# edwindn/rl-agent-for-qubit-array-tuning

Hardware: AMD Instinct MI355X
Metric: env steps/sec (batched 8-dot 64x64 CSD solves) (higher is better)
Workload: dtype f64; 1 GPU; 8-dot array, 4096 parallel envs per GPU, 64x64 CSD, deterministic physics (latching/noise off), 50-step episodes, staggered phases: 820 episode resets (new device + first observation) inside the timed region, synthetic CNN outputs; n_dots=8, envs_per_gpu=4096, resolution=64

## Files before the change

### __graft_entry__.py

```python
import os
import subprocess
import sys

ROOT = os.path.dirname(os.path.abspath(__file__))
PKG = os.path.join(ROOT, "rl-agent-for-qubit-array-tuning_amd")
for _p in (PKG, os.path.join(ROOT, "oracle"), os.path.join(ROOT, "tests")):
    if _p not in sys.path:
        sys.path.insert(0, _p)


def build() -> None:
    csrc = os.path.join(PKG, "csrc")
    subprocess.check_call(["make", "-C", csrc, "libqdsim.so"])
    subprocess.check_call(["make", "-C", os.path.join(ROOT, "tests", "hosttest"), "libqdsim_hosttest.so", "qd_scratch_asan"])
    subprocess.check_call(["make", "-C", os.path.join(ROOT, "tests", "hosttest_wave"), "libqdsim_hosttest_wave.so"])
    subprocess.check_call(["make", "-C", os.path.join(ROOT, "tests", "hosttest_gs"), "libqdsim_hosttest_gs.so"])
    subprocess.check_call(["make", "-C", os.path.join(ROOT, "tests", "hosttest_prune"), "libqdsim_hosttest_prune.so"])
    subprocess.check_call(["make", "-C", os.path.join(ROOT, "tests", "hosttest_points"), "libqdsim_hosttest_points.so"])
    subprocess.check_call(["make", "-C", os.path.join(ROOT, "tests", "hosttest_latch"), "libqdsim_hosttest_latch.so"])
    subprocess.check_call(["make", "-C", os.path.join(ROOT, "tests", "hosttest_scan"), "libqdsim_hosttest_scan.so"])
    subprocess.check_call(["make", "-C", os.path.join(ROOT, "tests", "hosttest_affine"), "libqdsim_hosttest_affine.so"])
    subprocess.check_call(["make", "-C", os.path.join(ROOT, "tests", "hosttest_line"), "libqdsim_hosttest_line.so"])
    subprocess.check_call(["make", "-C", os.path.join(ROOT, "tests", "hosttest_grid"), "libqdsim_hosttest_grid.so", "qd_grid_asan"])
    subprocess.check_call(["make", "-C", os.path.join(ROOT, "tests", "hosttest_tile"), "libqdsim_hosttest_tile.so", "qd_tile_asan"])
    subprocess.check_call(["make", "-C", os.path.join(ROOT, "tests", "hosttest_insert"), "all", "qd_insert_asan"])
    subprocess.check_call(["make", "-C", os.path.join(ROOT, "tests", "hosttest_closed"), "libqdsim_hosttest_closed.so", "qd_closed_asan"])
    subprocess.check_call(["make", "-C", os.path.join(ROOT, "tests", "hosttest_levels"), "libqdsim_hosttest_levels.so", "qd_levels_asan"])
    subprocess.check_call(["make", "-C", os.path.join(ROOT, "tests", "hosttest_thermal"), "libqdsim_hosttest_thermal.so", "qd_thermal_asan"])
    subprocess.check_call(["make", "-C", os.path.join(ROOT, "tests", "hosttest_thermal_blocks"), "libqdsim_hosttest_thermal_blocks.so",
                           "qd_thermal_blocks_asan"])
    subprocess.check_call(["make", "-C", os.path.join(ROOT, "tests", "hosttest_levels_blocks"), "libqdsim_hosttest_levels_blocks.so",
                           "qd_levels_blocks_asan"])
    subprocess.check_call(["make", "-C", os.path.join(ROOT, "tests", "hosttest_response"), "libqdsim_hosttest_response.so",
                           "qd_response_asan"])
    subprocess.check_call(["make", "-C", os.path.join(ROOT, "tests", "hosttest_response_blocks"), "libqdsim_hosttest_response_blocks.so",
                           "qd_response_blocks_asan"])
    subprocess.check_call(["make", "-C", os.path.join(ROOT, "tests", "gputest_eig"), "libqdsim_gputest_eig.so"])
    subprocess.check_call(["make", "-C", os.path.join(ROOT, "tests", "gputest_thermal_blocks"), "libqdsim_gputest_thermal_blocks.so"])
    subprocess.check_call(["make", "-C", os.path.join(ROOT, "tests", "gputest_levels_blocks"), "libqdsim_gputest_levels_blocks.so"])
    subprocess.check_call(["make", "-C", os.path.join(ROOT, "tests", "gputest_response"), "libqdsim_gputest_response.so"])
    subprocess.check_call(["make", "-C", os.path.join(ROOT, "tests", "gputest_response_blocks"), "libqdsim_gputest_response_blocks.so"])
    subprocess.check_call(["make", "-C", os.path.join(ROOT, "oracle"), "libqdoracle.so"])
    import qadapt_hip
    from qadapt_hip import _lib
    L = _lib.lib()
    missing = [n for n in _lib.EXPORTS + _lib.EXPORTS_WITH_DIGITS if not hasattr(L, n)]
    if missing:
        raise RuntimeError(f"libqdsim.so lacks symbols: {missing}")


def smoke() -> None:
    import numpy as np
    import torch
    import qd_oracle as O
    import helpers as H
    from qadapt_hip.vec_env import VecQuantumDeviceEnv, SyntheticCapacitanceModel

    assert torch.cuda.is_available(), "smoke() needs the MI355X"
    N, R, B, seed = 4, 16, 2, 2024
    env = VecQuantumDeviceEnv(B, num_dots=N, resolution=R, seed=seed, validate=True,
                              capacitance_model=SyntheticCapacitanceModel(3))
    rng = np.random.default_rng(0)
    C = N - 1
    v0 = rng.normal(0, 0.1, (B, C, 3)).astype(np.float32); l0 = rng.uniform(-6, -2, (B, C, 3)).astype(np.float32)
    obs = env.reset(cnn_outputs=(torch.as_tensor(v0).cuda(), torch.as_tensor(l0).cuda()))
    act = rng.uniform(-1, 1, (B, 2 * N - 1)).astype(np.float32)
    v1 = rng.normal(0, 0.1, (B, C, 3)).astype(np.float32); l1 = rng.uniform(-6, -2, (B, C, 3)).astype(np.float32)
    obs, rew, term, trunc = env.step(torch.as_tensor(act).cuda(),
                                     cnn_outputs=(torch.as_tensor(v1).cuda(), torch.as_tensor(l1).cuda()))
    img = obs["image"].cpu().numpy()
    raw, _ = env.raw()
    for e in range(B):
        oe = O.OracleEnv(N, R)
        oe.reset(O.sample_episode(np.random.default_rng(seed + e), N), v0[e], l0[e])
        oobs, (gr, br), _, _ = oe.step(act[e, :N], act[e, N:], v1[e], l1[e])
        r = rew[e].cpu().numpy()
        assert np.allclose(r[:N], gr, rtol=1e-9) and np.allclose(r[N:], br, rtol=1e-9), "reward mismatch"
        H.image_parity(oe, img[e], raw[e])
    env.close()
    print("smoke ok: 4-dot 16x16 batched step matches the oracle")


if __name__ == "__main__":
    build()
    if len(sys.argv) > 1 and sys.argv[1] == "smoke":
        smoke()
```

### rl-agent-for-qubit-array-tuning_amd/csrc/qd_tile.h

```cpp
#pragma once
#include "qd_pixel.h"
#include "qd_groundstate.h"

#define QD_FL_BIAS 0x7FFF
QD_HD bool qd_fl_packable(int fl) { return (unsigned)fl <= (unsigned)QD_FL_BIAS; }
QD_HD uint32_t qd_fl_pack(int fl) { return (uint32_t)fl | ((uint32_t)(QD_FL_BIAS - fl) << 16); }
QD_HD uint32_t qd_fl_pkmin(uint32_t a, uint32_t b) {
#if defined(__HIP_DEVICE_COMPILE__)
    typedef unsigned short u16x2 __attribute__((ext_vector_type(2)));
    return __builtin_bit_cast(uint32_t, __builtin_elementwise_min(__builtin_bit_cast(u16x2, a), __builtin_bit_cast(u16x2, b)));
#else
    const uint32_t la = a & 0xFFFFu, lb = b & 0xFFFFu, ha = a >> 16, hb = b >> 16;
    return (la < lb ? la : lb) | ((ha < hb ? ha : hb) << 16);
#endif
}
QD_HD void qd_fl_unpack(uint32_t w, int& mn, int& mx) { mn = (int)(w & 0xFFFFu); mx = QD_FL_BIAS - (int)(w >> 16); }

#ifndef QD_TILE_RESCAN8
#define QD_TILE_RESCAN8 1
#endif
template <int KC, bool FILL, bool RESCAN8 = (QD_TILE_RESCAN8 != 0)>
QD_HD void qd_tile_select(int nS, int nSfront, int scap, const uint32_t* scode, const double* sD, const double* sa, const double* sb,
                          double xs, double ys, uint32_t blo, uint32_t bhi, double* ke, uint16_t* kid,
                          double& maxE_out, int& maxS_out, int& maxG_out, int& count_out, double& eout_out) {
    constexpr int NG = KC / 8;
    double gE[4] = {-INFINITY, -INFINITY, -INFINITY, -INFINITY}; int gS[4] = {0, 8, 16, 24};
    double maxE = -INFINITY; int maxS = 0, maxG = 0, count = 0;
    double eout = INFINITY;
    int si0 = 0, nfree = 0;
    if (FILL && nSfront >= KC) {
#pragma unroll
        for (int g = 0; g < NG; ++g) {
            double me = -INFINITY; int ms = g * 8;
#pragma unroll
            for (int t = 0; t < 8; ++t) {
                const int s = g * 8 + t;
                const double en = fma(xs, sa[s], fma(ys, sb[s], sD[s]));
                ke[s * 64] = en; kid[s * 64] = (uint16_t)s;
                if (en > me) { me = en; ms = s; }
            }
            gE[g] = me; gS[g] = ms;
        }
        maxE = gE[0]; maxS = gS[0]; maxG = 0;
#pragma unroll
        for (int g = 1; g < NG; ++g) if (gE[g] > maxE) { maxE = gE[g]; maxS = gS[g]; maxG = g; }
        count = KC; si0 = KC; nfree = nSfront;
    }
    for (int si = si0; si < nS; ++si) {
        const int s = si < nSfront ? si : scap - 1 - (si - nSfront);
        const uint32_t code = scode[s];
        const bool valid = (si < nfree) ||
                           (((((code | 0x88888888u) - blo) & 0x88888888u) == 0x88888888u) &&
                            ((((bhi | 0x88888888u) - code) & 0x88888888u) == 0x88888888u));
        const double en = fma(xs, sa[s], fma(ys, sb[s], sD[s]));
        if (!valid) continue;
        if (count < KC) {
            ke[count * 64] = en; kid[count * 64] = (uint16_t)s;
            count++;
            if (count == KC) {
#pragma unroll
                for (int g = 0; g < NG; ++g) {
                    double me = -INFINITY; int ms = g * 8;
#pragma unroll
                    for (int t = 0; t < 8; ++t) { const double v = ke[(g * 8 + t) * 64]; if (v > me) { me = v; ms = g * 8 + t; } }
                    gE[g] = me; gS[g] = ms;
                }
                maxE = gE[0]; maxS = gS[0]; maxG = 0;
#pragma unroll
                for (int g = 1; g < NG; ++g) if (gE[g] > maxE) { maxE = gE[g]; maxS = gS[g]; maxG = g; }
            }
        } else if (en < maxE) {
            eout = fmin(eout, maxE);
            ke[maxS * 64] = en; kid[maxS * 64] = (uint16_t)s;
            {
                double me = -INFINITY; int ms = maxG * 8;
                if constexpr (RESCAN8) {
                    double v[8];
#pragma unroll
                    for (int t = 0; t < 8; ++t) v[t] = ke[(maxG * 8 + t) * 64];
#if defined(__HIP_DEVICE_COMPILE__)
                    __builtin_amdgcn_sched_barrier(0);
#endif
#pragma unroll
                    for (int t = 0; t < 8; ++t) if (v[t] > me) { me = v[t]; ms = maxG * 8 + t; }
                } else {
#pragma unroll
                    for (int t = 0; t < 8; ++t) { const double v = ke[(maxG * 8 + t) * 64]; if (v > me) { me = v; ms = maxG * 8 + t; } }
                }
#pragma unroll
                for (int g = 0; g < NG; ++g) if (g == maxG) { gE[g] = me; gS[g] = ms; }
            }
            maxE = gE[0]; maxS = gS[0]; maxG = 0;
#pragma unroll
            for (int g = 1; g < NG; ++g) if (gE[g] > maxE) { maxE = gE[g]; maxS = gS[g]; maxG = g; }
        } else {
            eout = fmin(eout, en);
        }
    }
    maxE_out = maxE; maxS_out = maxS; maxG_out = maxG; count_out = count; eout_out = eout;
}

#if defined(__HIPCC__)

#ifndef QD_TILE_PG_INTERLEAVED
#define QD_TILE_PG_INTERLEAVED 1
#endif
#ifndef QD_TILE_DPP
#define QD_TILE_DPP 1
#endif
#ifndef QD_TILE_FILL
#define QD_TILE_FILL 1
#endif

#ifndef QD_T_FCAP
#define QD_T_FCAP 832
#endif
#ifndef QD_T_SCAP
#define QD_T_SCAP 383
#endif
#define QD_T_REDO (-1)

struct QdTileLds {
    double m[QD_MAXN], g[QD_MAXN], lamx[QD_MAXN], lamy[QD_MAXN], tail[QD_MAXN], sla[QD_MAXN], slb[QD_MAXN], q[QD_MAXN];
    int lo[QD_MAXN], nd[QD_MAXN], cg[QD_MAXN];
    int optval[QD_MAXN][4];
    union {
        struct { double pn[2][QD_T_FCAP]; uint32_t code[2][QD_T_FCAP]; } f;
        struct { double e[QD_K][64]; uint16_t id[QD_K][64]; } k;
    } u;
    double sD[QD_T_SCAP], sa[QD_T_SCAP], sb[QD_T_SCAP];
    uint32_t scode[QD_T_SCAP];
#if defined(QD_TILE_PAD_LDS)
    char pad[QD_TILE_PAD_LDS];
#endif
};

__device__ __forceinline__ double qd_rl(double v, int lane) {
    const unsigned long long u = (unsigned long long)__double_as_longlong(v);
    const unsigned lo = (unsigned)__builtin_amdgcn_readlane((int)(unsigned)u, lane);
    const unsigned hi = (unsigned)__builtin_amdgcn_readlane((int)(unsigned)(u >> 32), lane);
    return __longlong_as_double((long long)(((unsigned long long)hi << 32) | lo));
}
template <int CTRL>
__device__ __forceinline__ int qd_dpp_i32(int v) { return __builtin_amdgcn_update_dpp(v, v, CTRL, 0xF, 0xF, false); }
#define QD_ROW_ALLREDUCE(v, OP, DPP)                                                                                   \
    v = OP(v, DPP<0xB1>(v));                                                               \
    v = OP(v, DPP<0x4E>(v));                                                               \
    v = OP(v, DPP<0x141>(v));                                                                     \
    v = OP(v, DPP<0x140>(v))
__device__ __forceinline__ int qd_wmin_i(int v) {
#if QD_TILE_DPP
    QD_ROW_ALLREDUCE(v, min, qd_dpp_i32);
    return min(min(__builtin_amdgcn_readlane(v, 0), __builtin_amdgcn_readlane(v, 16)),
               min(__builtin_amdgcn_readlane(v, 32), __builtin_amdgcn_readlane(v, 48)));
#else
#pragma unroll
    for (int o = 32; o > 0; o >>= 1) v = min(v, __shfl_xor(v, o, 64));
    return __builtin_amdgcn_readfirstlane(v);
#endif
}
__device__ __forceinline__ int qd_wmax_i(int v) {
#if QD_TILE_DPP
    QD_ROW_ALLREDUCE(v, max, qd_dpp_i32);
    return max(max(__builtin_amdgcn_readlane(v, 0), __builtin_amdgcn_readlane(v, 16)),
               max(__builtin_amdgcn_readlane(v, 32), __builtin_amdgcn_readlane(v, 48)));
#else
#pragma unroll
    for (int o = 32; o > 0; o >>= 1) v = max(v, __shfl_xor(v, o, 64));
    return __builtin_amdgcn_readfirstlane(v);
#endif
}
__device__ __forceinline__ double qd_wmin_d(double v) {
#if QD_TILE_DPP
    QD_ROW_ALLREDUCE(v, fmin, qd_dpp_f64);
    return fmin(fmin(qd_rl(v, 0), qd_rl(v, 16)), fmin(qd_rl(v, 32), qd_rl(v, 48)));
#else
#pragma unroll
    for (int o = 32; o > 0; o >>= 1) v = fmin(v, __shfl_xor(v, o, 64));
    return v;
#endif
}
__device__ __forceinline__ double qd_wmax_d(double v) {
#if QD_TILE_DPP
    QD_ROW_ALLREDUCE(v, fmax, qd_dpp_f64);
    return fmax(fmax(qd_rl(v, 0), qd_rl(v, 16)), fmax(qd_rl(v, 32), qd_rl(v, 48)));
#else
#pragma unroll
    for (int o = 32; o > 0; o >>= 1) v = fmax(v, __shfl_xor(v, o, 64));
    return v;
#endif
}
__device__ __forceinline__ void qd_wminmax_fl(int fl, int& mn, int& mx) {
    int v = (int)qd_fl_pack(fl);
#define QD_PKMIN_I(a, b) (int)qd_fl_pkmin((uint32_t)(a), (uint32_t)(b))
    QD_ROW_ALLREDUCE(v, QD_PKMIN_I, qd_dpp_i32);
#undef QD_PKMIN_I
    int lo = QD_FL_BIAS, hi = QD_FL_BIAS;
#pragma unroll
    for (int r = 0; r < 64; r += 16) {
        const unsigned w = (unsigned)__builtin_amdgcn_readlane(v, r);
        lo = min(lo, (int)(w & 0xFFFFu)); hi = min(hi, (int)(w >> 16));
    }
    mn = lo; mx = QD_FL_BIAS - hi;
}
__device__ __forceinline__ int qd_lane_prefix(unsigned long long mask) {
    return (int)__builtin_amdgcn_mbcnt_hi((unsigned)(mask >> 32), __builtin_amdgcn_mbcnt_lo((unsigned)mask, 0u));
}

__device__ __forceinline__ double qd_plane_max(double a, double b, double x0, double x1, double y0, double y1) {
    return fmax(x0 * a, x1 * a) + fmax(y0 * b, y1 * b);
}
__device__ __forceinline__ double qd_plane_min(double a, double b, double x0, double x1, double y0, double y1) {
    return fmin(x0 * a, x1 * a) + fmin(y0 * b, y1 * b);
}

template <int N>
__device__ __forceinline__ void qd_tile_point(const QdTileLds& T, const double* __restrict__ U, uint32_t code,
                                              double& pn, double& pa, double& pb) {
    double xv[N];
    pn = 0.0; pa = 0.0; pb = 0.0;
#pragma unroll
    for (int i = 0; i < N; ++i) {
        const int c = T.lo[i] + (int)((code >> (4 * (N - 1 - i))) & 15u);
        xv[i] = (double)c - T.m[i];
        double t = 0.0;
#pragma unroll
        for (int j = 0; j <= i; ++j) t = fma(U[j * N + i], xv[j], t);
        pn += fma(t, t, T.g[i] * xv[i]);
        const double dc = (double)(c - T.cg[i]);
        pa = fma(T.lamx[i], dc, pa);
        pb = fma(T.lamy[i], dc, pb);
    }
}

template <int N>
__device__ __forceinline__ void qd_tile_hand_over(QdPixelRec* rec, const double* vd, const double* ncont, double isa) {
#pragma unroll
    for (int i = 0; i < N; ++i) { rec->E[i] = ncont[i]; rec->E[8 + i] = vd[i]; }
    rec->E[16] = isa;
    rec->nvalid = QD_T_REDO;
}

template <int N, int KC, class FE = QdFrontEnv>
__global__ void __launch_bounds__(64)
qd_k_tile(const int* __restrict__ env_ids, int env_base, int R, const double* __restrict__ params,
          const double* __restrict__ state, QdPixelRec* __restrict__ recs, int sort_output, int noise_flags,
          unsigned long long* __restrict__ stats) {
    constexpr int G = N + 1, NB = N - 1, V = 2 * N;
    const QdLayout L = qd_layout(N);
    const int slot = blockIdx.z;
    const int e = env_ids ? env_ids[env_base + slot] : env_base + slot;
    const int ch = blockIdx.y;
    const int P = R * R;
    const int tiles_x = (R + 7) >> 3;
    const int ty = blockIdx.x / tiles_x, tx = blockIdx.x - ty * tiles_x;
    const int lane = threadIdx.x;
    const int px = tx * 8 + (lane & 7), py = ty * 8 + (lane >> 3);
    const bool inside = px < R && py < R;
    const int x = px < R ? px : R - 1, y = py < R ? py : R - 1;
    const int p = y * R + x;
    __shared__ QdTileLds T;
    const double* spar = params + (size_t)e * L.size;
    const double* sst = state + (size_t)e * L.s_size;
    if (qd_radial_replaced(spar, sst, L, ch, noise_flags)) return;
    QdPixelRec* rec = recs + ((size_t)slot * FE::channels(N) + ch) * P + p;
    const double* A = spar + L.cdd_inv;
    const double* U = spar + L.ufac;

    double vd[N], ncont[N], isa;
    double vpp[G], tc[NB];
    {
        double v_ext[V];
        FE::template voltages<N>(spar, sst, ch, R, x, y, v_ext, vpp, tc);
        if (inside) {
#pragma unroll
            for (int i = 0; i < G; ++i) rec->vpp[i] = vpp[i];
#pragma unroll
            for (int b = 0; b < NB; ++b) rec->tc[b] = tc[b];
        }
#pragma unroll
        for (int i = 0; i < N; ++i) vd[i] = vpp[i];
        qd_pixel_continuous<N, QD_TILE_PG_INTERLEAVED != 0>(spar, v_ext, vd, ncont, &isa);
    }
    int fl[N];
#pragma unroll
    for (int i = 0; i < N; ++i) fl[i] = (int)floor(ncont[i]);

#if defined(QD_TILE_STOP) && QD_TILE_STOP == 1
    if (inside) rec->E[0] = ncont[0] + vd[N - 1] + tc[0] + (double)fl[1];
    return;
#endif
    const int xr = min(tx * 8 + 3, R - 1), yr = min(ty * 8 + 3, R - 1);
    const double xs = (double)(x - xr), ys = (double)(y - yr);
    const double x0 = (double)(tx * 8 - xr), x1 = (double)(min(tx * 8 + 7, R - 1) - xr);
    const double y0 = (double)(ty * 8 - yr), y1 = (double)(min(ty * 8 + 7, R - 1) - yr);
    const double Xh = fmax(-x0, x1), Yh = fmax(-y0, y1);
    bool fail = false;
    int why = 0;
    double rho;
    double v0[N];
    {
        double r1 = 0.0;
        double dxv[N], dyv[N], mref[N];
#pragma unroll
        for (int i = 0; i < N; ++i) {
            v0[i] = qd_rl(vd[i], 27);
            mref[i] = qd_rl(ncont[i], 27);
            dxv[i] = qd_rl(vd[i], 1) - qd_rl(vd[i], 0);
            dyv[i] = qd_rl(vd[i], 8) - qd_rl(vd[i], 0);
            const double r = ((vd[i] - v0[i]) - xs * dxv[i]) - ys * dyv[i];
            r1 += fabs(r);
            if (lane == 0) T.m[i] = mref[i];
        }
        double colsum = 0.0;
        {
            const int row = lane < N ? lane : 0;
            double tg = 0.0, tx_ = 0.0, ty_ = 0.0;
#pragma unroll
            for (int j = 0; j < N; ++j) {
                const double a = A[row * G + j];
                tg = fma(a, mref[j] - v0[j], tg);
                tx_ = fma(a, dxv[j], tx_);
                ty_ = fma(a, dyv[j], ty_);
                colsum += fabs(a);
            }
            if (lane < N) { T.g[lane] = 2.0 * tg; T.lamx[lane] = -2.0 * tx_; T.lamy[lane] = -2.0 * ty_; }
        }
        const double anorm = qd_wmax_d(lane < N ? colsum : 0.0);
        rho = qd_wmax_d(r1) * anorm;
    }
    int lo_[N], alo_[N], ahi_[N], nd_[N];
    unsigned long long allvalid_count = 1;
#if QD_TILE_DPP
    bool packed;
    {
        int orfl = 0;
#pragma unroll
        for (int i = 0; i < N; ++i) orfl |= fl[i];
        packed = __ballot(!qd_fl_packable(orfl)) == 0ull;
    }
#endif
#pragma unroll
    for (int i = 0; i < N; ++i) {
        int fmn, fmx;
#if QD_TILE_DPP
        if (packed) qd_wminmax_fl(fl[i], fmn, fmx);
        else
#endif
        { fmn = qd_wmin_i(fl[i]); fmx = qd_wmax_i(fl[i]); }
        lo_[i] = max(fmn - 1, 0); const int hi = fmx + 2;
        alo_[i] = max(fmx - 1, 0); ahi_[i] = fmn + 2;
        nd_[i] = hi - lo_[i] + 1;
        if (nd_[i] > 8 || ahi_[i] < alo_[i]) { fail = true; why = 1; }
        allvalid_count *= (unsigned long long)(ahi_[i] >= alo_[i] ? ahi_[i] - alo_[i] + 1 : 0);
        if (lane == 0) { T.lo[i] = lo_[i]; T.nd[i] = nd_[i]; }
    }
    static_assert(KC == 8 || KC == 16 || KC == 32, "kept sets come in groups of 8");
    if (allvalid_count < (unsigned long long)KC) { fail = true; why = 1; }
    __builtin_amdgcn_wave_barrier();

#if defined(QD_TILE_STOP) && QD_TILE_STOP == 2
    if (inside) rec->E[0] = rho + v0[0];
    return;
#endif
    double Tpp = INFINITY, pn_ref = 0.0, margin = 0.0, Ecg = 0.0;
    if (!fail) {
        int cg[N];
        {
            double dm[N];
#pragma unroll
            for (int i = 0; i < N; ++i) {
                double s = 0.0;
#pragma unroll
                for (int j = 0; j < i; ++j) s = fma(U[j * N + i], dm[j], s);
                const double ui = spar[L.uinv + i];
                const double cstar = T.m[i] + fma(-s, ui, -(0.5 * T.g[i]) * (ui * ui));
                double c = rint(cstar);
                c = fmin(fmax(c, (double)alo_[i]), (double)ahi_[i]);
                if (!(c == c)) c = (double)alo_[i];
                cg[i] = (int)c; dm[i] = c - T.m[i];
                if (lane == 0) { T.cg[i] = cg[i]; T.optval[i][0] = cg[i]; }
            }
            {
                const int row = lane < N ? lane : 0;
                double t = 0.0;
#pragma unroll
                for (int j = 0; j < N; ++j) t = fma(A[row * G + j], (double)cg[j] - v0[j], t);
                if (lane < N) T.q[lane] = t;
            }
        }
        __builtin_amdgcn_wave_barrier();
        {
            double dd[N];
#pragma unroll
            for (int i = 0; i < N; ++i) dd[i] = (double)cg[i] - vd[i];
            double E = 0.0;
#pragma unroll 1
            for (int i = 0; i < N; ++i) {
                const double t = qd_dotN<N>(A + i * G, dd);
                double di = dd[0];
#pragma unroll
                for (int j = 1; j < N; ++j) di = (j == i) ? dd[j] : di;
                E = fma(di, t, E);
            }
            Ecg = E;
        }
        {
            double acc = 0.0, sa = 0.0, sb = 0.0;
#pragma unroll
            for (int j = N - 1; j >= 0; --j) {
                if (lane == 0) { T.tail[j] = acc; T.sla[j] = sa; T.slb[j] = sb; }
                const double gj = T.g[j], mj = T.m[j];
                const double cmin = (double)lo_[j], cmax = (double)(lo_[j] + nd_[j] - 1);
                acc += fmin(gj * (cmin - mj), gj * (cmax - mj));
                const double span = fmax((double)(cg[j] - lo_[j]), (double)(lo_[j] + nd_[j] - 1 - cg[j]));
                sa += fabs(T.lamx[j]) * span; sb += fabs(T.lamy[j]) * span;
            }
        }
        double cost = INFINITY; int oi = lane >> 3, oc = 0;
        {
            int a_lo = 0, a_hi = -1, cgi = 0;
#pragma unroll
            for (int i = 0; i < N; ++i) if (i == oi) { a_lo = alo_[i]; a_hi = ahi_[i]; cgi = cg[i]; }
            oc = a_lo + (lane & 7);
            if (oi < N && oc <= a_hi && oc != cgi) {
                const double dc = (double)(oc - cgi);
                cost = fma(2.0 * dc, T.q[oi], A[oi * G + oi] * dc * dc);
            }
        }
        int nopt[N];
#pragma unroll
        for (int i = 0; i < N; ++i) nopt[i] = 1;
        int prod = 1;
        for (int it = 0; it < 24; ++it) {
            const double mn = qd_wmin_d(cost);
            if (!(mn < INFINITY)) break;
            const unsigned long long who = __ballot(cost == mn);
            const int wl = __builtin_ctzll(who);
            const int wi = wl >> 3;
            int ni = 1;
#pragma unroll
            for (int i = 0; i < N; ++i) if (i == wi) ni = nopt[i];
            const int wc = __builtin_amdgcn_readlane(oc, wl);
            if (ni < 4 && (prod / ni) * (ni + 1) <= 64) {
                if (lane == 0) T.optval[wi][ni] = wc;
#pragma unroll
                for (int i = 0; i < N; ++i) if (i == wi) nopt[i] = ni + 1;
                prod = (prod / ni) * (ni + 1);
            }
            if (lane == wl) cost = INFINITY;
        }
        __builtin_amdgcn_wave_barrier();
        uint32_t scode_seed = 0;
        {
            int rem = lane;
#pragma unroll
            for (int i = N - 1; i >= 0; --i) {
                const int sel = rem % nopt[i]; rem /= nopt[i];
                const int c = T.optval[i][sel];
                scode_seed |= (uint32_t)(c - lo_[i]) << (4 * (N - 1 - i));
            }
        }
        double pn, pa, pb;
        qd_tile_point<N>(T, U, scode_seed, pn, pa, pb);
        pn_ref = qd_rl(pn, 0);
        const double escale = qd_wmax_d(fabs(pn)) + fabs(pn_ref) + 1.0;
        int maxdc = 0;
#pragma unroll
        for (int i = 0; i < N; ++i) maxdc = max(maxdc, max(cg[i] - lo_[i], lo_[i] + nd_[i] - 1 - cg[i]));
        margin = 2.0 * rho * (double)maxdc + 1e-11 * escale + 1e-12 * qd_wmax_d(fabs(Ecg));
        const double Mh = (lane < prod) ? (pn - pn_ref) + qd_plane_max(pa, pb, x0, x1, y0, y1) + margin : INFINITY;
        if (prod < KC) { fail = true; why = 2; }
        else {
            int below = 0;
            for (int j = 0; j < 64; ++j) {
                const double o = qd_rl(Mh, j);
                below += (o < Mh || (o == Mh && j < lane)) ? 1 : 0;
            }
            const unsigned long long sel = __ballot(below == KC - 1 && lane < prod);
            Tpp = sel ? qd_rl(Mh, __builtin_ctzll(sel)) : INFINITY;
            if (!(Tpp < INFINITY)) { fail = true; why = 2; }
        }
    }

#if defined(QD_TILE_STOP) && QD_TILE_STOP == 3
    if (inside) rec->E[0] = Tpp + pn_ref + margin + Ecg;
    return;
#endif
    int nfront = 0, cur = 0;
    if (!fail) {
        if (lane == 0) { T.u.f.pn[0][0] = 0.0; T.u.f.code[0][0] = 0u; }
        nfront = 1;
        __builtin_amdgcn_wave_barrier();
#pragma unroll 1
        for (int i = 0; i < N && !fail; ++i) {
            const double mi = T.m[i], gi = T.g[i], lxi = T.lamx[i], lyi = T.lamy[i];
            const double tl = T.tail[i], sla = T.sla[i], slb = T.slb[i];
            const double uii = U[i * N + i];
            const int loi = T.lo[i], ndi = T.nd[i], cgi = T.cg[i];
            const unsigned sh = 4u * (unsigned)(N - 1 - i);
            int nout = 0;
#pragma unroll 1
            for (int base = 0; base < nfront; base += 64) {
                const int node = base + lane;
                const bool act = node < nfront;
                const uint32_t code = act ? T.u.f.code[cur][node] : 0u;
                const double pn0 = act ? T.u.f.pn[cur][node] : 0.0;
                double s = 0.0, pa0 = 0.0, pb0 = 0.0;
#pragma unroll 1
                for (int j = 0; j < i; ++j) {
                    const int c = T.lo[j] + (int)((code >> (4 * (N - 1 - j))) & 15u);
                    s = fma(U[j * N + i], (double)c - T.m[j], s);
                    const double dc = (double)(c - T.cg[j]);
                    pa0 = fma(T.lamx[j], dc, pa0); pb0 = fma(T.lamy[j], dc, pb0);
                }
#pragma unroll 1
                for (int k = 0; k < ndi; ++k) {
                    const double xk = (double)(loi + k) - mi;
                    const double t = fma(uii, xk, s);
                    const double pn2 = pn0 + fma(t, t, gi * xk);
                    const double dc = (double)(loi + k - cgi);
                    const double pa2 = fma(lxi, dc, pa0), pb2 = fma(lyi, dc, pb0);
                    const double W = fma(Xh, fabs(pa2) + sla, Yh * (fabs(pb2) + slb));
                    const double LB = ((pn2 - pn_ref) + tl) - W - margin;
                    const bool keep = act && (LB <= Tpp);
                    const unsigned long long km = __ballot(keep);
                    const int pos = nout + qd_lane_prefix(km);
                    if (keep && pos < QD_T_FCAP) {
                        T.u.f.pn[cur ^ 1][pos] = pn2;
                        T.u.f.code[cur ^ 1][pos] = code | ((uint32_t)k << sh);
                    }
                    nout += __builtin_popcountll(km);
                }
            }
            if (nout > QD_T_FCAP) { fail = true; why = 3; }
            nfront = nout; cur ^= 1;
            __builtin_amdgcn_wave_barrier();
        }
    }

#if defined(QD_TILE_STOP) && QD_TILE_STOP == 4
    if (inside) rec->E[0] = (double)nfront + T.u.f.pn[cur][lane];
    return;
#endif
    int nS = 0, nSfront = 0;
    if (!fail && nfront < KC) { fail = true; why = 4; }
    if (!fail) {
        constexpr int CH = QD_T_FCAP / 64;
        double Mh[CH];
        uint32_t vlo = 0, vhi = 0;
#pragma unroll
        for (int i = 0; i < N; ++i) {
            vlo |= (uint32_t)(alo_[i] - lo_[i]) << (4 * (N - 1 - i));
            vhi |= (uint32_t)(ahi_[i] - lo_[i]) << (4 * (N - 1 - i));
        }
        double mlo = INFINITY;
#pragma unroll
        for (int c = 0; c < CH; ++c) {
            Mh[c] = INFINITY;
            const int node = c * 64 + lane;
            if (c * 64 < nfront && node < nfront) {
                const uint32_t code = T.u.f.code[cur][node];
                const bool av = ((((code | 0x88888888u) - vlo) & 0x88888888u) == 0x88888888u) &&
                                ((((vhi | 0x88888888u) - code) & 0x88888888u) == 0x88888888u);
                if (av) {
                    double pn, pa, pb;
                    qd_tile_point<N>(T, U, code, pn, pa, pb);
                    Mh[c] = (pn - pn_ref) + qd_plane_max(pa, pb, x0, x1, y0, y1) + margin;
                }
                mlo = fmin(mlo, Mh[c]);
            }
        }
        double tlo = qd_wmin_d(mlo), thi = Tpp;
        for (int it = 0; it < 14; ++it) {
            const double mid = 0.5 * (tlo + thi);
            int cnt = 0;
#pragma unroll
            for (int c = 0; c < CH; ++c) cnt += __builtin_popcountll(__ballot(Mh[c] <= mid));
            if (cnt >= KC) thi = mid; else tlo = mid;
        }
        const double Tt = thi;
        int nfrontS = 0, nbackS = 0;
#pragma unroll 1
        for (int c = 0; c < CH; ++c) {
            if (c * 64 >= nfront) break;
            const int node = c * 64 + lane;
            bool take = false, likely = false;
            uint32_t code = 0; double D = 0.0, pa = 0.0, pb = 0.0;
            if (node < nfront) {
                code = T.u.f.code[cur][node];
                double pn;
                qd_tile_point<N>(T, U, code, pn, pa, pb);
                D = pn - pn_ref;
                take = (D + qd_plane_min(pa, pb, x0, x1, y0, y1) - margin) <= Tt;
                double mhc = INFINITY;
#pragma unroll
                for (int cc = 0; cc < CH; ++cc) if (cc == c) mhc = Mh[cc];
                likely = take && (mhc <= Tt);
            }
            const unsigned long long kf = __ballot(likely), kb = __ballot(take && !likely);
            const int tot = nfrontS + nbackS + __builtin_popcountll(kf) + __builtin_popcountll(kb);
            if (tot <= QD_T_SCAP) {
                int pos = -1;
                if (likely) pos = nfrontS + qd_lane_prefix(kf);
                else if (take) pos = QD_T_SCAP - 1 - (nbackS + qd_lane_prefix(kb));
                if (pos >= 0) { T.scode[pos] = code; T.sD[pos] = D; T.sa[pos] = pa; T.sb[pos] = pb; }
            }
            nfrontS += __builtin_popcountll(kf); nbackS += __builtin_popcountll(kb);
        }
        nS = nfrontS + nbackS;
        nSfront = nfrontS;
        if (nS > QD_T_SCAP || nS < KC) { fail = true; why = 5; }
        __builtin_amdgcn_wave_barrier();
    }
    if (stats && lane == 0) {
        atomicAdd(&stats[0], 1ull);
        if (fail) { atomicAdd(&stats[1], 1ull); atomicAdd(&stats[8 + why], 1ull); }
        atomicAdd(&stats[3], (unsigned long long)nS);
    }
    if (fail) {
        if (inside) qd_tile_hand_over<N>(rec, vd, ncont, isa);
        return;
    }

#if defined(QD_TILE_STOP) && QD_TILE_STOP == 5
    if (inside) rec->E[0] = (double)nS + T.sD[lane];
    return;
#endif
    uint32_t blo = 0, bhi = 0;
#pragma unroll
    for (int i = 0; i < N; ++i) {
        blo |= (uint32_t)(max(fl[i] - 1, 0) - lo_[i]) << (4 * (N - 1 - i));
        bhi |= (uint32_t)(fl[i] + 2 - lo_[i]) << (4 * (N - 1 - i));
    }
    double maxE, eout; int maxS, maxG, count;
    qd_tile_select<KC, QD_TILE_FILL != 0>(nS, nSfront, QD_T_SCAP, T.scode, T.sD, T.sa, T.sb, xs, ys, blo, bhi, &T.u.k.e[0][lane],
                                          &T.u.k.id[0][lane], maxE, maxS, maxG, count, eout);
    const double amb = 2.0 * margin;
    const bool redo = (count < KC) || !(eout - maxE > amb);
    if (stats) {
        const unsigned long long rm = __ballot(redo && inside), rc = __ballot(count < KC && inside);
        if (lane == 0 && rm) { atomicAdd(&stats[2], (unsigned long long)__builtin_popcountll(rm)); atomicAdd(&stats[4], (unsigned long long)__builtin_popcountll(rc)); }
    }
    if (!inside) return;
    if (redo) { qd_tile_hand_over<N>(rec, vd, ncont, isa); return; }

#if defined(QD_TILE_STOP) && QD_TILE_STOP == 6
    if (inside) rec->E[0] = maxE + eout + (double)count;
    return;
#endif
    {
    uint32_t off = 0;
#pragma unroll
    for (int i = 0; i < N; ++i) off |= (uint32_t)(lo_[i] - fl[i] + 1 + 4) << (4 * (N - 1 - i));
    if (sort_output) {
        for (int k = 0; k < KC; ++k) {
            const uint32_t code = T.scode[T.u.k.id[k][lane]];
            double dd[N];
#pragma unroll
            for (int i = 0; i < N; ++i) dd[i] = (double)(lo_[i] + (int)((code >> (4 * (N - 1 - i))) & 15u)) - vd[i];
            double E = 0.0;
#pragma unroll 1
            for (int i = 0; i < N; ++i) {
                const double t = qd_dotN<N>(A + i * G, dd);
                double di = dd[0];
#pragma unroll
                for (int j = 1; j < N; ++j) di = (j == i) ? dd[j] : di;
                E = fma(di, t, E);
            }
            T.u.k.e[k][lane] = E;
        }
        for (int i = 1; i < KC; ++i) {
            const double E = T.u.k.e[i][lane]; const uint16_t id = T.u.k.id[i][lane];
            const uint32_t cd = T.scode[id];
            int pos = i;
            while (pos > 0) {
                const double ep = T.u.k.e[pos - 1][lane]; const uint16_t ip = T.u.k.id[pos - 1][lane];
                const bool less = (E < ep) || (E == ep && cd < T.scode[ip]);
                if (!less) break;
                T.u.k.e[pos][lane] = ep; T.u.k.id[pos][lane] = ip;
                --pos;
            }
            T.u.k.e[pos][lane] = E; T.u.k.id[pos][lane] = id;
        }
    }
    double e1 = INFINITY, e2 = INFINITY;
    for (int k = 0; k < KC; ++k) {
        const uint32_t code = T.scode[T.u.k.id[k][lane]];
        const uint32_t dg = (code + off) - 0x44444444u;
        unsigned idx = dg & 0x33333333u;
        idx = (idx | (idx >> 2)) & 0x0F0F0F0Fu;
        idx = (idx | (idx >> 4)) & 0x00FF00FFu;
        idx = (idx | (idx >> 8)) & 0x0000FFFFu;
        rec->idx[k] = (uint16_t)idx;
        const double ek = T.u.k.e[k][lane];
        e2 = fmin(e2, fmax(e1, ek)); e1 = fmin(e1, ek);
        const double E = sort_output ? ek : ek + Ecg;
        rec->E[k] = E * isa;
    }
    if (!sort_output && !(e2 - e1 > amb)) { qd_tile_hand_over<N>(rec, vd, ncont, isa); return; }
#pragma unroll
    for (int i = 0; i < N; ++i) rec->fl[i] = fl[i];
    rec->nvalid = KC;
    }
}

#endif
```

Baseline: 14700 env-steps/s.

## Reuse stored leaf energies and add early exits in tile option/front expansion

```diff
diff --git a/__graft_entry__.py b/__graft_entry__.py
--- a/__graft_entry__.py
+++ b/__graft_entry__.py
@@ -23,6 +23,8 @@
     subprocess.check_call(["make", "-C", os.path.join(ROOT, "tests", "hosttest_line"), "libqdsim_hosttest_line.so"])
     subprocess.check_call(["make", "-C", os.path.join(ROOT, "tests", "hosttest_grid"), "libqdsim_hosttest_grid.so", "qd_grid_asan"])
     subprocess.check_call(["make", "-C", os.path.join(ROOT, "tests", "hosttest_tile"), "libqdsim_hosttest_tile.so", "qd_tile_asan"])
+    subprocess.check_call(["make", "-C", os.path.join(ROOT, "tests", "hosttest_tile_uniform"), "libqdsim_hosttest_tile_uniform.so",
+                           "qd_tile_uniform_asan"])
     subprocess.check_call(["make", "-C", os.path.join(ROOT, "tests", "hosttest_insert"), "all", "qd_insert_asan"])
     subprocess.check_call(["make", "-C", os.path.join(ROOT, "tests", "hosttest_closed"), "libqdsim_hosttest_closed.so", "qd_closed_asan"])
     subprocess.check_call(["make", "-C", os.path.join(ROOT, "tests", "hosttest_levels"), "libqdsim_hosttest_levels.so", "qd_levels_asan"])
diff --git a/rl-agent-for-qubit-array-tuning_amd/csrc/qd_tile.h b/rl-agent-for-qubit-array-tuning_amd/csrc/qd_tile.h
--- a/rl-agent-for-qubit-array-tuning_amd/csrc/qd_tile.h
+++ b/rl-agent-for-qubit-array-tuning_amd/csrc/qd_tile.h
@@ -98,6 +98,50 @@
         }
     }
     maxE_out = maxE; maxS_out = maxS; maxG_out = maxG; count_out = count; eout_out = eout;
+}
+
+#ifndef QD_TILE_OPT_EXIT
+#define QD_TILE_OPT_EXIT 1
+#endif
+#ifndef QD_TILE_OVF_EXIT
+#define QD_TILE_OVF_EXIT 1
+#endif
+#ifndef QD_TILE_LEAF_PN
+#define QD_TILE_LEAF_PN 1
+#endif
+
+QD_HD bool qd_tile_opt_open(int prod, int ni) { return ni < 4 && prod * (ni + 1) <= 64 * ni; }
+template <int N>
+QD_HD bool qd_tile_opt_any_open(const int* nopt, int prod) {
+    bool open = false;
+#pragma unroll
+    for (int i = 0; i < N; ++i) open = open || qd_tile_opt_open(prod, nopt[i]);
+    return open;
+}
+
+template <int N>
+QD_HD void qd_tile_level_term(uint32_t code, int j, double u, double m, int lo, int cg, double lamx, double lamy,
+                              double& s, double& pa0, double& pb0) {
+    const int c = lo + (int)((code >> (4 * (N - 1 - j))) & 15u);
+    s = fma(u, (double)c - m, s);
+    const double dc = (double)(c - cg);
+    pa0 = fma(lamx, dc, pa0); pb0 = fma(lamy, dc, pb0);
+}
+QD_HD double qd_tile_child_pn(double pn0, double s, double uii, double xk, double gi) {
+    const double t = fma(uii, xk, s);
+    return pn0 + fma(t, t, gi * xk);
+}
+template <int N>
+QD_HD void qd_tile_point_ab(const int* lo, const int* cg, const double* lamx, const double* lamy, uint32_t code,
+                            double& pa, double& pb) {
+    pa = 0.0; pb = 0.0;
+#pragma unroll
+    for (int i = 0; i < N; ++i) {
+        const int c = lo[i] + (int)((code >> (4 * (N - 1 - i))) & 15u);
+        const double dc = (double)(c - cg[i]);
+        pa = fma(lamx[i], dc, pa);
+        pb = fma(lamy[i], dc, pb);
+    }
 }
 
 #if defined(__HIPCC__)
@@ -432,7 +476,12 @@
 #pragma unroll
         for (int i = 0; i < N; ++i) nopt[i] = 1;
         int prod = 1;
+#if QD_TILE_OPT_EXIT
+        bool open = true;
+        for (int it = 0; it < 24 && open; ++it) {
+#else
         for (int it = 0; it < 24; ++it) {
+#endif
             const double mn = qd_wmin_d(cost);
             if (!(mn < INFINITY)) break;
             const unsigned long long who = __ballot(cost == mn);
@@ -442,12 +491,24 @@
 #pragma unroll
             for (int i = 0; i < N; ++i) if (i == wi) ni = nopt[i];
             const int wc = __builtin_amdgcn_readlane(oc, wl);
+#if QD_TILE_OPT_EXIT
+            if (qd_tile_opt_open(prod, ni)) {
+                if (lane == 0) T.optval[wi][ni] = wc;
+#pragma unroll
+                for (int i = 0; i < N; ++i) if (i == wi) nopt[i] = ni + 1;
+                prod = 1;
+#pragma unroll
+                for (int i = 0; i < N; ++i) prod *= nopt[i];
+                open = qd_tile_opt_any_open<N>(nopt, prod);
+            }
+#else
             if (ni < 4 && (prod / ni) * (ni + 1) <= 64) {
                 if (lane == 0) T.optval[wi][ni] = wc;
 #pragma unroll
                 for (int i = 0; i < N; ++i) if (i == wi) nopt[i] = ni + 1;
                 prod = (prod / ni) * (ni + 1);
             }
+#endif
             if (lane == wl) cost = INFINITY;
         }
         __builtin_amdgcn_wave_barrier();
@@ -508,17 +569,12 @@
                 const double pn0 = act ? T.u.f.pn[cur][node] : 0.0;
                 double s = 0.0, pa0 = 0.0, pb0 = 0.0;
 #pragma unroll 1
-                for (int j = 0; j < i; ++j) {
-                    const int c = T.lo[j] + (int)((code >> (4 * (N - 1 - j))) & 15u);
-                    s = fma(U[j * N + i], (double)c - T.m[j], s);
-                    const double dc = (double)(c - T.cg[j]);
-                    pa0 = fma(T.lamx[j], dc, pa0); pb0 = fma(T.lamy[j], dc, pb0);
-                }
+                for (int j = 0; j < i; ++j)
+                    qd_tile_level_term<N>(code, j, U[j * N + i], T.m[j], T.lo[j], T.cg[j], T.lamx[j], T.lamy[j], s, pa0, pb0);
 #pragma unroll 1
                 for (int k = 0; k < ndi; ++k) {
                     const double xk = (double)(loi + k) - mi;
-                    const double t = fma(uii, xk, s);
-                    const double pn2 = pn0 + fma(t, t, gi * xk);
+                    const double pn2 = qd_tile_child_pn(pn0, s, uii, xk, gi);
                     const double dc = (double)(loi + k - cgi);
                     const double pa2 = fma(lxi, dc, pa0), pb2 = fma(lyi, dc, pb0);
                     const double W = fma(Xh, fabs(pa2) + sla, Yh * (fabs(pb2) + slb));
@@ -532,6 +588,9 @@
                     }
                     nout += __builtin_popcountll(km);
                 }
+#if QD_TILE_OVF_EXIT
+                if (nout > QD_T_FCAP) break;
+#endif
             }
             if (nout > QD_T_FCAP) { fail = true; why = 3; }
             nfront = nout; cur ^= 1;
@@ -565,7 +624,12 @@
                                 ((((vhi | 0x88888888u) - code) & 0x88888888u) == 0x88888888u);
                 if (av) {
                     double pn, pa, pb;
+#if QD_TILE_LEAF_PN
+                    pn = T.u.f.pn[cur][node];
+                    qd_tile_point_ab<N>(T.lo, T.cg, T.lamx, T.lamy, code, pa, pb);
+#else
                     qd_tile_point<N>(T, U, code, pn, pa, pb);
+#endif
                     Mh[c] = (pn - pn_ref) + qd_plane_max(pa, pb, x0, x1, y0, y1) + margin;
                 }
                 mlo = fmin(mlo, Mh[c]);
@@ -590,7 +654,12 @@
             if (node < nfront) {
                 code = T.u.f.code[cur][node];
                 double pn;
+#if QD_TILE_LEAF_PN
+                pn = T.u.f.pn[cur][node];
+                qd_tile_point_ab<N>(T.lo, T.cg, T.lamx, T.lamy, code, pa, pb);
+#else
                 qd_tile_point<N>(T, U, code, pn, pa, pb);
+#endif
                 D = pn - pn_ref;
                 take = (D + qd_plane_min(pa, pb, x0, x1, y0, y1) - margin) <= Tt;
                 double mhc = INFINITY;
```

Result: faster. 14920 env-steps/s (median of 6 runs) (+1.5%).
